# zju3dv/neuralbody

Hardware: NVIDIA H100
Metric: rays_per_s_512x512_64spp (higher is better)
Workload: dtype f16x2 (hi+lo fp16 pairs, fp32 accumulate)

## Files before the change

### neuralbody_b200/csrc/nb_render_tc_list.cu

```cuda
#include "nb_tc_common.cuh"
#include <type_traits>

namespace nb {
namespace tcl {

using tcr::Quad;

constexpr int TP = 128;
constexpr int NUM_SEGS = 6;
constexpr int MAXS = 1024;
constexpr uint32_t ID_MASK = 0x0FFFFFFFu;

__device__ __forceinline__ unsigned long long global_ns() {
    unsigned long long t;
    asm volatile("mov.u64 %0, %%globaltimer;" : "=l"(t));
    return t;
}

__device__ __forceinline__ void load_frame_xf(const RenderParams& P, FrameXf* xf, int i) {
    const int b = P.frame;
    if (i < 9) xf->R[i] = __ldg(P.R + b * 9 + i);
    if (i < 3) {
        xf->Th[i] = __ldg(P.Th + b * 3 + i);
        xf->min_dhw[i] = __ldg(P.bounds + b * 6 + (2 - i));
// ... 61 lines not shown
#pragma unroll
        for (int c = 0; c < 4; ++c) {
            const uint32_t bal = __ballot_sync(0xffffffffu, cls[k] == c);
            if (lane == 0) wcnt[c][slot] = __popc(bal);
        }
    }
    __syncthreads();
    if (tid < 4) {
        int total = 0;
        for (int w = 0; w < MAXS / 32; ++w) total += wcnt[tid][w];
        stotal[tid] = total;
        sbase[tid] = total ? atomicAdd(P.list_count + tid, (unsigned int)total) : 0u;
    }
    __syncthreads();
    const float4 empty = make_float4(0.f, 0.f, 0.f, fminf(sigma_empty, 0.f));
#pragma unroll
    for (int k = 0; k < CLS_PER_THREAD; ++k) {
        const int slot = k * (CLS_THREADS / 32) + warp;
        const int c = cls[k];
        const uint32_t same = __match_any_sync(0xffffffffu, c);
        if (c >= 0) {
            int local = __popc(same & ((1u << lane) - 1));
            for (int w = 0; w < slot; ++w) local += wcnt[c][w];
            float4* buf = c >= 2 ? P.list_a : P.list_b;
            const size_t at = (c & 1) ? (size_t)sbase[c] + local : P.list_cap - (size_t)sbase[c] - stotal[c] + local;
            buf[at] = gm[k];
        } else if (live[k]) {
            P.raw_ws[(__float_as_uint(gm[k].w) & ID_MASK) - id0] = empty;
        }
    }
}

constexpr int NT = 384;
constexpr int NROWT = 96;
constexpr int LAUNCH_REGS = (65536 / NT) / 8 * 8;
constexpr int PRODUCER_REGS = 56, CONSUMER_REGS = 224;
constexpr int CHUNK_STRIDE = TP * 16 + 16;
constexpr int ACT_CHUNKS = kHidden / 8;
constexpr int PLANE_BYTES = ACT_CHUNKS * CHUNK_STRIDE;
constexpr int SEG_BUFS = 4;
constexpr int SLOT_BYTES = 16384, NUM_SLOTS = 4;
constexpr int TILE256 = kHalfTile256 * 2;
constexpr int TILE3 = kHalfTile3 * 2;
constexpr int L3_PUSH = 4;
constexpr int L3_PUSHES = (kStepsL3 + L3_PUSH - 1) / L3_PUSH;
constexpr int HEAD_FLOATS = kHidden + 4 + 3 * kColor + 4 + 3 * kHidden;
constexpr int H_ALPHA = 0, H_RGBW = kHidden + 4, H_RGBB = H_RGBW + 3 * kColor, H_B0 = H_RGBB + 4;
constexpr int OFF_HI = 0, OFF_LO = PLANE_BYTES;
constexpr int OFF_RING = 2 * PLANE_BYTES;
constexpr int OFF_HEAD = OFF_RING + NUM_SLOTS * SLOT_BYTES;
constexpr int OFF_XF = OFF_HEAD + HEAD_FLOATS * 4;
constexpr int OFF_SCHED = OFF_XF + 128;
constexpr int OFF_ROWS = OFF_SCHED + 64;
constexpr int OFF_BAR = OFF_ROWS + 2 * TP * 16;
enum { B_FULL = 0, B_EMPTY = B_FULL + NUM_SLOTS, B_ROWSFULL = B_EMPTY + NUM_SLOTS, B_L2DONE, B_PEFULL, NUM_BARS };
constexpr int SMEM_BYTES = OFF_BAR + NUM_BARS * 8;
static_assert(SMEM_BYTES <= 232448, "shared memory budget");
static_assert(OFF_RING % 128 == 0 && OFF_HEAD % 16 == 0 && OFF_ROWS % 16 == 0 && OFF_BAR % 8 == 0, "alignment");
static_assert(128 * PRODUCER_REGS + 256 * CONSUMER_REGS <= NT * LAUNCH_REGS, "register pool of the CTA");

__host__ __device__ constexpr int pushes_per_tile(int l0_ksteps) { return l0_ksteps + 2 * kKsL12 + L3_PUSHES; }

__device__ __forceinline__ uint32_t act_off(int row, int k) {
    return (uint32_t)((k >> 3) * CHUNK_STRIDE + (row >> 3) * 128 + (row & 7) * 16 + (k & 7) * 2);
}

template <int NP, typename VT>
__global__ void __launch_bounds__(NT, 1) render_tc_list_kernel(const __grid_constant__ RenderParams P) {
    extern __shared__ __align__(1024) unsigned char smem[];
    uint64_t* bars = reinterpret_cast<uint64_t*>(smem + OFF_BAR);
    FrameXf* xf = reinterpret_cast<FrameXf*>(smem + OFF_XF);
    float* head = reinterpret_cast<float*>(smem + OFF_HEAD);
    float4* rows_buf = reinterpret_cast<float4*>(smem + OFF_ROWS);
    const int tid = threadIdx.x, lane = tid & 31;
    const int warp = __shfl_sync(0xffffffffu, tid >> 5, 0);
    const int wgid = warp >> 2;
    const int S = P.n_samples;
    const uint32_t s_hi0 = tc::smem_u32(smem + OFF_HI), s_lo0 = tc::smem_u32(smem + OFF_LO), s_ring = tc::smem_u32(smem + OFF_RING);

    if (tid == 0) {
        for (int i = 0; i < NUM_SLOTS; ++i) {
            tc::mbar_init(&bars[B_FULL + i], 1);
            tc::mbar_init(&bars[B_EMPTY + i], 8);
        }
        tc::mbar_init(&bars[B_ROWSFULL], NROWT);
        tc::mbar_init(&bars[B_L2DONE], 8);
        tc::mbar_init(&bars[B_PEFULL], NROWT);
        tc::fence_mbar_init();
    }
    load_frame_xf(P, xf, tid);
    for (int i = tid; i < HEAD_FLOATS; i += NT) {
        float v;
        if (i < H_RGBW) v = __ldg(P.wf32 + oAlphaW + i);
        else if (i < H_B0) v = __ldg(P.wf32 + oRgbW + (i - H_RGBW));
        else {
            const int j = i - H_B0, l = j / kHidden, n = j % kHidden;
            v = __ldg(P.wf32 + (l == 0 ? oB0 : l == 1 ? oB1 : oB2) + n);
        }
        head[i] = v;
    }
    struct Sched { unsigned int cnt[4]; int start[4]; int n_tiles; };
    Sched* sched = reinterpret_cast<Sched*>(smem + OFF_SCHED);
    if (tid == 0) {
        int acc = 0;
        for (int c = 0; c < 4; ++c) {
            const unsigned int n = P.list_count[c];
            sched->cnt[c] = n;
            sched->start[c] = acc;
            acc += (int)((n + TP - 1) / TP);
        }
        sched->n_tiles = acc;
        if (P.stats) atomicMax(P.frame_clock + 0, ~global_ns());
    }
    __syncthreads();
    const int n_tiles = sched->n_tiles;
    struct TileRef { int cls, nrows; const float4* ent; };
    auto tile_ref = [&](int tile) {
        TileRef r;
        r.cls = tile >= sched->start[3] ? 3 : tile >= sched->start[2] ? 2 : tile >= sched->start[1] ? 1 : 0;
        const int lt = tile - sched->start[r.cls];
        const unsigned int cnt = sched->cnt[r.cls];
        const long long rem = (long long)cnt - (long long)lt * TP;
        r.nrows = rem <= 0 ? 0 : rem < TP ? (int)rem : TP;
        const float4* buf = r.cls >= 2 ? P.list_a : P.list_b;
        r.ent = buf + ((r.cls & 1) ? (size_t)0 : P.list_cap - (size_t)cnt) + (size_t)lt * TP;
        return r;
    };

    if (wgid == 0) {
        tc::setmaxnreg_dec<PRODUCER_REGS>();
        const uint32_t s_hi = s_hi0, s_lo = s_lo0;
        if (warp == 0) {
            if (lane == 0) {
                tcr::Tracer tl;
                tl.init(P.trace, 3);
                const unsigned char* seq = reinterpret_cast<const unsigned char*>(P.wf16);
                unsigned long long real_tiles = 0, real_ksteps = 0;
                uint32_t g = 0;
                for (int tile = blockIdx.x; tile < n_tiles; tile += gridDim.x) {
                    const TileRef tref = tile_ref(tile);
                    const int l0_ksteps = class_ksteps(tref.cls);
                    real_tiles += tref.nrows > 0;
                    real_ksteps += tref.nrows > 0 ? l0_ksteps : 0;
                    for (int j = 0; j < pushes_per_tile(l0_ksteps); ++j, ++g) {
                        const uint32_t slot = g % NUM_SLOTS;
                        tc::mbar_wait(&bars[B_EMPTY + slot], ((g / NUM_SLOTS) & 1) ^ 1);
                        if (j == 0) tl.ev(1);
                        unsigned char* dst = smem + OFF_RING + slot * SLOT_BYTES;
                        uint64_t* bar = &bars[B_FULL + slot];
                        if (j < l0_ksteps + 2 * kKsL12) {
                            const int layer = j < l0_ksteps ? 0 : j < l0_ksteps + kKsL12 ? 1 : 2;
                            const int ks = layer == 0 ? j : layer == 1 ? j - l0_ksteps : j - l0_ksteps - kKsL12;
                            const int nks = layer == 0 ? kKsL0 : kKsL12;
                            const unsigned char* base = seq + 2 * (layer == 0 ? sL0 : layer == 1 ? sL1 : sL2);
                            tc::mbar_arrive_expect_tx(bar, (uint32_t)(2 * (NP == 3 ? 2 : 1) * TILE256));
#pragma unroll
                            for (int h = 0; h < 2; ++h)
#pragma unroll
                                for (int pl = 0; pl < (NP == 3 ? 2 : 1); ++pl)
                                    tc::bulk_g2s(dst + (2 * h + pl) * TILE256, base + 2 * pair_step_offset(ks, pl, h, nks), TILE256, bar);
                        } else {
                            const int g0 = (j - l0_ksteps - 2 * kKsL12) * L3_PUSH;
                            const int n = min(L3_PUSH, kStepsL3 - g0), common = min(n, kStepsL3 - 1 - g0);
                            const bool last = g0 + n == kStepsL3;
                            tc::mbar_arrive_expect_tx(bar, (uint32_t)(2 * n * TILE3));
#pragma unroll
                            for (int h = 0; h < 2; ++h) {
                                unsigned char* d = dst + h * (SLOT_BYTES / 2);
                                tc::bulk_g2s(d, seq + 2 * (sL3 + pair_l3_offset(g0, h)), common * TILE3, bar);
                                if (last)
                                    tc::bulk_g2s(d + common * TILE3, reinterpret_cast<const unsigned char*>(P.wframe) + ((size_t)P.frame * 2 + h) * TILE3,
                                                 TILE3, bar);
                            }
                        }
                    }
                    tl.ev(2);
                }
                if (P.stats) {
                    atomicAdd(P.stats + 0, real_tiles);
                    atomicAdd(P.stats + 4, real_ksteps);
                    if (blockIdx.x == 0) atomicAdd(P.stats + 1, (unsigned long long)sched->cnt[0] + sched->cnt[1] + sched->cnt[2] + sched->cnt[3]);
                }
            }
            __syncwarp();
        } else {
            const int pt = tid - 32;
            tcr::Tracer tr;
            tr.init(pt == 0 ? P.trace : nullptr, 0);
            auto pwait = [&](uint64_t* bar, uint32_t parity) { tc::mbar_wait_backoff(bar, parity, 64); };
            auto load_rows = [&](float4* dst, int tile) {
                if (tile < n_tiles) {
                    const TileRef r = tile_ref(tile);
                    for (int i = pt; i < TP; i += NROWT)
                        dst[i] = i < r.nrows ? __ldg(r.ent + i) : make_float4(0.f, 0.f, 0.f, __uint_as_float(0xFFFFFFFFu));
                }
                tcr::named_bar_sync(3, NROWT);
                tc::mbar_arrive(&bars[B_ROWSFULL]);
            };

            load_rows(rows_buf, blockIdx.x);
            int it = 0;
            for (int tile = blockIdx.x; tile < n_tiles; tile += gridDim.x, ++it) {
                const TileRef tref = tile_ref(tile);
                const int nrows = tref.nrows;
                const float4* rows = rows_buf + (it & 1) * TP;
                tr.ev(1);

                pwait(&bars[B_L2DONE], it & 1);
                tr.ev(31);
#pragma unroll 1
                for (int job = pt; job < 2 * TP; job += NROWT) {
                    const int prow = job % TP;
                    const float4 e = rows[prow];
                    auto put = [&](int k, float v) {
                        const __half hv = __float2half_rn(v);
                        asm volatile("st.shared.b16 [%0], %1;" ::"r"(s_lo + act_off(prow, k)), "h"(*reinterpret_cast<const unsigned short*>(&hv)) : "memory");
                    };
                    if (job < TP) {
                        positional_embed_anchored<10, 5>(e.x, e.y, e.z, [&](int j, float v) { put(j, v); });
                        put(63, 0.f);
                    } else {
                        const int smp = (int)(__float_as_uint(e.w) & ID_MASK);
                        const size_t ri = (size_t)P.frame * P.n_rays + (prow < nrows ? smp / S : 0);
                        const float dx = __ldg(P.ray_d + ri * 3), dy = __ldg(P.ray_d + ri * 3 + 1), dz = __ldg(P.ray_d + ri * 3 + 2);
                        const float nrm = sqrtf(__fadd_rn(__fadd_rn(__fmul_rn(dx, dx), __fmul_rn(dy, dy)), __fmul_rn(dz, dz)));
                        positional_embed_anchored<4, 4>(__fdiv_rn(dx, nrm), __fdiv_rn(dy, nrm), __fdiv_rn(dz, nrm), [&](int j, float v) { put(64 + j, v); });
                        put(91, 0.f); put(92, 1.f); put(93, 1.f); put(94, 0.f); put(95, 0.f);
                    }
                }
                tc::fence_proxy_async();
                tc::mbar_arrive(&bars[B_PEFULL]);
                tr.ev(32);
                load_rows(rows_buf + ((it + 1) & 1) * TP, tile + gridDim.x);
                tr.ev(30);
            }
        }
    } else {
        tc::setmaxnreg_inc<CONSUMER_REGS>();
        uint32_t s_hi, s_lo;
        const int cw = wgid - 1;
        const bool arr = lane == 0;
        tcr::Tracer tr;
        tr.init((tid & 127) == 0 ? P.trace : nullptr, 1 + cw);
        const int r0 = 64 * cw + 16 * (warp & 3) + (lane >> 2), cq = 2 * (lane & 3);
        float acc0[64], acc1[64];
        auto init_bias = [&](const float* b) {
#pragma unroll
            for (int c = 0; c < 16; ++c) {
                const float2 v0 = *reinterpret_cast<const float2*>(b + 8 * c + cq), v1 = *reinterpret_cast<const float2*>(b + 128 + 8 * c + cq);
                acc0[4 * c] = v0.x; acc0[4 * c + 1] = v0.y; acc0[4 * c + 2] = v0.x; acc0[4 * c + 3] = v0.y;
                acc1[4 * c] = v1.x; acc1[4 * c + 1] = v1.y; acc1[4 * c + 2] = v1.x; acc1[4 * c + 3] = v1.y;
            }
        };
        const uint32_t wg_rows = (uint32_t)(cw * 8 * 128);
        auto mma256 = [&](uint32_t slot, int ka) {
            const uint64_t a_hi = tc::make_smem_desc(s_hi + wg_rows + 2 * ka * CHUNK_STRIDE, CHUNK_STRIDE, 128);
            const uint64_t a_lo = tc::make_smem_desc(s_lo + wg_rows + 2 * ka * CHUNK_STRIDE, CHUNK_STRIDE, 128);
            const uint64_t b0h = tc::make_smem_desc(slot + 0 * TILE256, 128 * 16, 128);
            const uint64_t b0l = tc::make_smem_desc(slot + 1 * TILE256, 128 * 16, 128);
            const uint64_t b1h = tc::make_smem_desc(slot + 2 * TILE256, 128 * 16, 128);
            const uint64_t b1l = tc::make_smem_desc(slot + 3 * TILE256, 128 * 16, 128);
            tc::wgmma_m64n128k16_f16(acc0, a_hi, b0h, true);
            tc::wgmma_m64n128k16_f16(acc1, a_hi, b1h, true);
            if (NP == 3) {
                tc::wgmma_m64n128k16_f16(acc0, a_lo, b0h, true);
                tc::wgmma_m64n128k16_f16(acc1, a_lo, b1h, true);
                tc::wgmma_m64n128k16_f16(acc0, a_hi, b0l, true);
                tc::wgmma_m64n128k16_f16(acc1, a_hi, b1l, true);
            }
        };
        uint32_t g = 0;
        uint32_t w_stall = 0, r_stall = 0, pe_stall = 0, g_cycles = 0;
        auto take = [&](auto&& mma) {
            const uint32_t s = g % NUM_SLOTS;
            const uint32_t t0 = (uint32_t)clock();
            tc::mbar_wait(&bars[B_FULL + s], (g / NUM_SLOTS) & 1);
            w_stall += (uint32_t)clock() - t0;
            tc::wgmma_fence();
            mma(s_ring + s * SLOT_BYTES);
            tc::wgmma_commit();
            ++g;
        };
        auto release = [&](uint32_t gp, bool pred) { tc::mbar_arrive_if(&bars[B_EMPTY + gp % NUM_SLOTS], pred); };
        auto release_last = [&]() { release(g - 1, arr); };

        auto convert = [&](bool last) {
            float sig0 = 0.f, sig1 = 0.f;
            auto one = [&](const float (&a)[64], int nh) {
#pragma unroll
                for (int c = 0; c < 16; ++c) {
                    const int col = 128 * nh + 8 * c + cq;
#pragma unroll
                    for (int hr = 0; hr < 2; ++hr) {
                        const float x0 = a[4 * c + 2 * hr], x1 = a[4 * c + 2 * hr + 1];
                        const uint32_t off = act_off(r0 + 8 * hr, col);
                        uint32_t hv;
                        if (last) {
                            const float2 aw = *reinterpret_cast<const float2*>(head + H_ALPHA + col);
                            float& sg = hr ? sig1 : sig0;
                            sg = fmaf(fmaxf(x0, 0.f), aw.x, sg);
                            sg = fmaf(fmaxf(x1, 0.f), aw.y, sg);
                            hv = tc::cvt_relu_f16x2(x0, x1);
                        } else if (NP == 3) {
                            hv = tc::cvt_rz_relu_f16x2(x0, x1);
                            float q0, q1;
                            tc::trunc_residual2(x0, x1, q0, q1);
                            const uint32_t lv = tc::cvt_relu_f16x2(q0, q1);
                            asm volatile("st.shared.b32 [%0], %1;" ::"r"(s_lo + off), "r"(lv) : "memory");
                        } else {
                            hv = tc::cvt_relu_f16x2(x0, x1);
                        }
                        asm volatile("st.shared.b32 [%0], %1;" ::"r"(s_hi + off), "r"(hv) : "memory");
                    }
                }
            };
            one(acc0, 0);
            one(acc1, 1);
            return make_float2(sig0, sig1);
        };
        auto publish = [&]() {
            tc::fence_proxy_async();
            tcr::named_bar_sync(1 + cw, 128);
        };

        int it = 0;
        for (int tile = blockIdx.x; tile < n_tiles; tile += gridDim.x, ++it) {
            const TileRef tref = tile_ref(tile);
            const int nrows = tref.nrows, nseg = class_segments(tref.cls);
            const float4* rows = rows_buf + (it & 1) * TP;
            asm volatile("mov.u32 %0, %1;" : "=r"(s_hi) : "r"(s_hi0));
            asm volatile("mov.u32 %0, %1;" : "=r"(s_lo) : "r"(s_lo0));
            tr.ev(1);
            auto gather = [&](int seg) {
                const unsigned char* volbase = reinterpret_cast<const unsigned char*>(P.volume);
                const int grp = (tid & 127) >> 3, t = tid & 7;
                const int lvl = seg < 2 ? 3 : seg < 4 ? 2 : seg < 5 ? 1 : 0;
                const int cbase0 = seg < 2 ? seg * 64 : seg < 4 ? (seg - 2) * 64 : 0;
                const int nunits = seg == NUM_SEGS - 1 ? 1 : 2;
                const int C = P.lvl_C[lvl], D = P.lvl_D[lvl], H = P.lvl_H[lvl], W = P.lvl_W[lvl];
                const unsigned char* lvl_ptr = volbase + P.lvl_off[lvl] + ((size_t)P.frame * P.lvl_bstride[lvl] + 4 * t) * sizeof(VT);
                const uint32_t dX = (uint32_t)(C * sizeof(VT)), dY = dX * W, dZ = dY * H;
                const int kb = 64 * (seg % SEG_BUFS);
                for (int row = 64 * cw + grp; row < 64 * cw + 64; row += 16) {
                    const float4 e = rows[row];
                    const bool occ = row < nrows && ((__float_as_uint(e.w) >> (28 + lvl)) & 1u);
                    float acc[2][4] = {{0.f, 0.f, 0.f, 0.f}, {0.f, 0.f, 0.f, 0.f}};
                    if (occ) {
                        float gx, gy, gz;
                        world_to_grid(*xf, e.x, e.y, e.z, gx, gy, gz);
                        Corners cn;
                        corner_setup(unnormalize(gx, W), unnormalize(gy, H), unnormalize(gz, D), W, H, D, cn);
                        auto axis = [](int i0, int size, float (&w)[2]) {
                            if (i0 < 0) { w[0] = w[1]; w[1] = 0.f; return 0; }
                            if (i0 >= size) { w[0] = w[1] = 0.f; return size - 2; }
                            if (i0 == size - 1) { w[1] = w[0]; w[0] = 0.f; return size - 2; }
                            return i0;
                        };
                        const int xc = axis(cn.x0, W, cn.wx), yc = axis(cn.y0, H, cn.wy), zc = axis(cn.z0, D, cn.wz);
                        const uint32_t cb = (uint32_t)((zc * H + yc) * W + xc) * dX;
                        float cw[8];
#pragma unroll
                        for (int c = 0; c < 8; ++c) cw[c] = __fmul_rn(__fmul_rn(cn.wx[c & 1], cn.wy[(c >> 1) & 1]), cn.wz[c >> 2]);
#pragma unroll
                        for (int uu = 0; uu < 2; ++uu) {
                            if (uu >= nunits) continue;
                            const unsigned char* ub = lvl_ptr + (size_t)(cbase0 + 32 * uu) * sizeof(VT);
                            typename Quad<VT>::raw v[8];
#pragma unroll
                            for (int c = 0; c < 8; ++c)
                                v[c] = Quad<VT>::load_bytes(ub + cb + ((c & 1) ? dX : 0u) + ((c & 2) ? dY : 0u) + ((c & 4) ? dZ : 0u));
#pragma unroll
                            for (int c = 0; c < 8; ++c)
                                if (cw[c] != 0.f) Quad<VT>::fma(acc[uu], v[c], cw[c]);
                        }
                    }
#pragma unroll
                    for (int uu = 0; uu < 2; ++uu) {
                        if (uu >= nunits) continue;
                        const float (&a)[4] = acc[uu];
                        const uint32_t off = act_off(row, kb + 32 * uu + 4 * t);
                        uint2 hw, lw;
                        if (NP == 3) {
                            hw.x = tc::cvt_rz_f16x2(a[0], a[1]); hw.y = tc::cvt_rz_f16x2(a[2], a[3]);
                            float q0, q1, q2, q3;
                            tc::trunc_residual2(a[0], a[1], q0, q1);
                            tc::trunc_residual2(a[2], a[3], q2, q3);
                            lw.x = tc::cvt_f16x2(q0, q1); lw.y = tc::cvt_f16x2(q2, q3);
                            tcr::sts_v2(s_lo + off, lw);
                        } else {
                            hw.x = tc::cvt_f16x2(a[0], a[1]); hw.y = tc::cvt_f16x2(a[2], a[3]);
                        }
                        tcr::sts_v2(s_hi + off, hw);
                    }
                }
            };

            {
                const uint32_t t0 = (uint32_t)clock();
                tc::mbar_wait(&bars[B_ROWSFULL], it & 1);
                r_stall += (uint32_t)clock() - t0;
            }
            init_bias(head + H_B0);
            for (int seg = 0; seg < nseg; ++seg) {
                const uint32_t t0 = (uint32_t)clock();
                gather(seg);
                publish();
                g_cycles += (uint32_t)clock() - t0;
                const int nks = seg == NUM_SEGS - 1 ? 2 : 4, ka = 4 * (seg % SEG_BUFS);
                for (int q = 0; q < nks; ++q) {
                    take([&](uint32_t slot) { mma256(slot, ka + q); });
                    tc::wgmma_wait<1>();
                    tc::acc_fence(acc0); tc::acc_fence(acc1);
                    release(g - 2, arr && q > 0);
                }
                tc::wgmma_wait<0>();
                tc::acc_fence(acc0); tc::acc_fence(acc1);
                release_last();
            }
            tr.ev(20);
            convert(false);
            init_bias(head + H_B0 + kHidden);
            publish();
            float2 sig = make_float2(0.f, 0.f);
            for (int layer = 1; layer <= 2; ++layer) {
                for (int q = 0; q < kKsL12; ++q) {
                    take([&](uint32_t slot) { mma256(slot, q); });
                    tc::wgmma_wait<1>();
                    tc::acc_fence(acc0); tc::acc_fence(acc1);
                    release(g - 2, arr && q > 0);
                }
                tc::wgmma_wait<0>();
                tc::acc_fence(acc0); tc::acc_fence(acc1);
                release_last();
                tr.ev(20 + layer);
                if (layer == 1) {
                    convert(false);
                    init_bias(head + H_B0 + 2 * kHidden);
                } else {
                    tc::mbar_arrive_if(&bars[B_L2DONE], arr);
                    sig = convert(true);
                }
                publish();
            }
            float c3a[32], c3b[32];
#pragma unroll
            for (int i = 0; i < 32; ++i) { c3a[i] = 0.f; c3b[i] = 0.f; }
#pragma unroll
            for (int p = 0; p < L3_PUSHES; ++p) {
                if (p * L3_PUSH == 16) {
                    const uint32_t t0 = (uint32_t)clock();
                    tc::mbar_wait(&bars[B_PEFULL], it & 1);
                    pe_stall += (uint32_t)clock() - t0;
                }
                take([&](uint32_t slot) {
#pragma unroll
                    for (int k = 0; k < L3_PUSH; ++k) {
                        const int ks = p * L3_PUSH + k;
                        if (ks >= kStepsL3) break;
                        const uint32_t a = ks < 16 ? s_hi + 2 * ks * CHUNK_STRIDE : s_lo + 2 * (ks - 16) * CHUNK_STRIDE;
                        const uint64_t ad = tc::make_smem_desc(a + wg_rows, CHUNK_STRIDE, 128);
                        tc::wgmma_m64n64k16_f16(c3a, ad, tc::make_smem_desc(slot + k * TILE3, 64 * 16, 128), true);
                        tc::wgmma_m64n64k16_f16(c3b, ad, tc::make_smem_desc(slot + SLOT_BYTES / 2 + k * TILE3, 64 * 16, 128), true);
                    }
                });
                tc::wgmma_wait<1>();
                tc::acc_fence(c3a); tc::acc_fence(c3b);
                release(g - 2, arr && p > 0);
            }
            tc::wgmma_wait<0>();
            tc::acc_fence(c3a); tc::acc_fence(c3b);
            release_last();
            tr.ev(23);
            float cr[2] = {0.f, 0.f}, cg[2] = {0.f, 0.f}, cbl[2] = {0.f, 0.f};
            auto color = [&](const float (&a)[32], int nh) {
#pragma unroll
                for (int c = 0; c < 8; ++c) {
                    const int col = 64 * nh + 8 * c + cq;
                    const float2 w0 = *reinterpret_cast<const float2*>(head + H_RGBW + col);
                    const float2 w1 = *reinterpret_cast<const float2*>(head + H_RGBW + kColor + col);
                    const float2 w2 = *reinterpret_cast<const float2*>(head + H_RGBW + 2 * kColor + col);
#pragma unroll
                    for (int hr = 0; hr < 2; ++hr) {
                        const float x0 = fmaxf(a[4 * c + 2 * hr], 0.f), x1 = fmaxf(a[4 * c + 2 * hr + 1], 0.f);
                        cr[hr] = fmaf(x1, w0.y, fmaf(x0, w0.x, cr[hr]));
                        cg[hr] = fmaf(x1, w1.y, fmaf(x0, w1.x, cg[hr]));
                        cbl[hr] = fmaf(x1, w2.y, fmaf(x0, w2.x, cbl[hr]));
                    }
                }
            };
            color(c3a, 0);
            color(c3b, 1);
            float sg[2] = {sig.x, sig.y};
#pragma unroll
            for (int hr = 0; hr < 2; ++hr) {
#pragma unroll
                for (int o = 1; o <= 2; o <<= 1) {
                    cr[hr] += __shfl_xor_sync(0xffffffffu, cr[hr], o);
                    cg[hr] += __shfl_xor_sync(0xffffffffu, cg[hr], o);
                    cbl[hr] += __shfl_xor_sync(0xffffffffu, cbl[hr], o);
                    sg[hr] += __shfl_xor_sync(0xffffffffu, sg[hr], o);
                }
                const int row = r0 + 8 * hr;
                if ((lane & 3) == 0 && row < nrows) {
                    const int smp = (int)(__float_as_uint(rows[row].w) & ID_MASK);
                    P.raw_ws[smp] = make_float4(cr[hr] + head[H_RGBB], cg[hr] + head[H_RGBB + 1], cbl[hr] + head[H_RGBB + 2],
                                                sg[hr] + head[H_ALPHA + kHidden]);
                }
            }
            tr.ev(24);
            tr.val(50, w_stall);
            tr.val(51, r_stall);
            tr.val(52, pe_stall);
            tr.val(53, g_cycles);
            w_stall = r_stall = pe_stall = g_cycles = 0;
        }
    }
    __syncthreads();
    if (tid == 0 && P.stats) atomicMax(P.frame_clock + 1, global_ns());
}

constexpr int COMP_WARPS = 8;
__global__ void __launch_bounds__(COMP_WARPS * 32) composite_kernel(const __grid_constant__ RenderParams P) {
    __shared__ float zs[COMP_WARPS][MAXS];
    const int warp = threadIdx.x >> 5, lane = threadIdx.x & 31;
    const int ray = blockIdx.x * COMP_WARPS + warp;
    if (blockIdx.x == 0 && threadIdx.x == 0 && P.stats) {
        const unsigned long long t0 = ~P.frame_clock[0], t1 = P.frame_clock[1];
        atomicAdd(P.stats + 2, t1 > t0 ? t1 - t0 : 0ull);
        atomicAdd(P.stats + 3, 1ull);
    }
    if (ray >= P.n_rays) return;
    const int S = P.n_samples;
    const size_t rg = (size_t)P.frame * P.n_rays + ray;
    const float near = __ldg(P.near + rg), far = __ldg(P.far + rg);
    for (int s = lane; s < S; s += 32) zs[warp][s] = z_sample(near, far, P.t_vals, s, S, P.t_rand ? P.t_rand + rg * S : nullptr, P.z_user ? P.z_user + rg * S : nullptr);
    __syncwarp();
    const float dx = __ldg(P.ray_d + rg * 3), dy = __ldg(P.ray_d + rg * 3 + 1), dz = __ldg(P.ray_d + rg * 3 + 2);
    const float nrm = sqrtf(__fadd_rn(__fadd_rn(__fmul_rn(dx, dx), __fmul_rn(dy, dy)), __fmul_rn(dz, dz)));
    float* wout = P.weights ? P.weights + rg * S : nullptr;
    RayOut o = composite_ray(P.raw_ws + (size_t)ray * S, zs[warp], S, nrm, wout, lane);
    if (lane == 0) {
        const float add = P.white_bkgd ? __fsub_rn(1.f, o.acc) : 0.f;
        P.rgb_map[rg * P.rgb_stride + 0] = o.r + add;
        P.rgb_map[rg * P.rgb_stride + 1] = o.g + add;
        P.rgb_map[rg * P.rgb_stride + 2] = o.b + add;
        P.depth_map[rg * P.map_stride] = o.depth;
        P.acc_map[rg * P.map_stride] = o.acc;
        P.disp_map[rg * P.map_stride] = disparity(o.depth, o.acc);
    }
}

template <int NP, typename VT>
static cudaError_t launch_list(const RenderParams& p, int grid, cudaStream_t stream) {
    cudaError_t e = cudaFuncSetAttribute(render_tc_list_kernel<NP, VT>, cudaFuncAttributeMaxDynamicSharedMemorySize, SMEM_BYTES);
    if (e != cudaSuccess) return e;
    render_tc_list_kernel<NP, VT><<<grid, NT, SMEM_BYTES, stream>>>(p);
    return cudaGetLastError();
}

static size_t align256(size_t v) { return (v + 255) & ~(size_t)255; }
constexpr size_t CTL_BYTES = 32;

}

bool tc_available() { return true; }

size_t render_tc_list_workspace_bytes(int batch, int n_rays, int n_samples) {
    const size_t per_frame = (size_t)n_rays * n_samples * sizeof(float4);
    return tcl::align256((size_t)batch * tcl::CTL_BYTES) + 3 * tcl::align256(per_frame);
}

// ... 70 lines not shown
```

### neuralbody_b200/csrc/nb_tc_common.cuh

```cuda
#pragma once
#include "nb_device.cuh"
#include "nb_tc_ptx.cuh"

namespace nb {
namespace tcr {

__device__ __forceinline__ void named_bar_sync(int id, int nthreads) {
    asm volatile("bar.sync %0, %1;" ::"r"(id), "r"(nthreads) : "memory");
}
__device__ __forceinline__ uint4 ldg_nc_v4(const void* p) {
    uint4 r;
    asm volatile("ld.global.nc.v4.u32 {%0,%1,%2,%3}, [%4];" : "=r"(r.x), "=r"(r.y), "=r"(r.z), "=r"(r.w) : "l"(p));
    return r;
}
__device__ __forceinline__ void sts_v2(uint32_t addr, uint2 v) {
    asm volatile("st.shared.v2.b32 [%0], {%1, %2};" ::"r"(addr), "r"(v.x), "r"(v.y) : "memory");
}
__device__ __forceinline__ float f16lo_of(float x, uint32_t hi_pair, int which) {
    const __half2 h = *reinterpret_cast<const __half2*>(&hi_pair);
    return x - (which ? __high2float(h) : __low2float(h));
}

struct Tracer {
    unsigned long long* buf;
    int n;
    __device__ __forceinline__ void init(unsigned long long* base, int role) {
        buf = (base && blockIdx.x == 0) ? base + role * 4096 : nullptr;
        n = 0;
    }
    __device__ __forceinline__ void ev(int code) { val(code, (unsigned long long)clock64()); }
    __device__ __forceinline__ void val(int code, unsigned long long v) {
        if (buf && n < 4096) buf[n++] = ((unsigned long long)code << 48) | (v & 0xFFFFFFFFFFFFull);
    }
};

template <typename VT> struct Quad;
template <> struct Quad<float> {
    using raw = uint4;
    static __device__ __forceinline__ raw zero() { return make_uint4(0u, 0u, 0u, 0u); }
    static __device__ __forceinline__ raw load(const float* p) { return ldg_nc_v4(p); }
    static __device__ __forceinline__ raw load_bytes(const unsigned char* p) { return ldg_nc_v4(p); }
    static __device__ __forceinline__ void fma(float (&a)[4], const raw& v, float w) {
        a[0] = fmaf(__uint_as_float(v.x), w, a[0]); a[1] = fmaf(__uint_as_float(v.y), w, a[1]);
        a[2] = fmaf(__uint_as_float(v.z), w, a[2]); a[3] = fmaf(__uint_as_float(v.w), w, a[3]);
    }
};
template <> struct Quad<__half> {
    using raw = uint2;
    static __device__ __forceinline__ raw zero() { return make_uint2(0u, 0u); }
    static __device__ __forceinline__ raw load(const __half* p) {
        uint2 r;
        asm volatile("ld.global.nc.v2.u32 {%0,%1}, [%2];" : "=r"(r.x), "=r"(r.y) : "l"(p));
        return r;
    }
    static __device__ __forceinline__ raw load_bytes(const unsigned char* p) { return load(reinterpret_cast<const __half*>(p)); }
    static __device__ __forceinline__ void fma(float (&a)[4], const raw& v, float w) {
        const float2 f0 = __half22float2(*reinterpret_cast<const __half2*>(&v.x));
        const float2 f1 = __half22float2(*reinterpret_cast<const __half2*>(&v.y));
        a[0] = fmaf(f0.x, w, a[0]); a[1] = fmaf(f0.y, w, a[1]);
        a[2] = fmaf(f1.x, w, a[2]); a[3] = fmaf(f1.y, w, a[3]);
    }
};

}
}
```

### neuralbody_b200/csrc/nb_tc_ptx.cuh

```cuda
#pragma once
#include <cuda_fp16.h>
#include <stdint.h>

namespace nb {
namespace tc {

__device__ __forceinline__ uint32_t smem_u32(const void* p) { return (uint32_t)__cvta_generic_to_shared(p); }

__device__ __forceinline__ void mbar_init(uint64_t* bar, uint32_t count) {
    asm volatile("mbarrier.init.shared::cta.b64 [%0], %1;" ::"r"(smem_u32(bar)), "r"(count));
}
__device__ __forceinline__ void fence_mbar_init() { asm volatile("fence.mbarrier_init.release.cluster;" ::: "memory"); }
__device__ __forceinline__ void mbar_arrive(uint64_t* bar) {
    asm volatile("{\n\t.reg .b64 st;\n\tmbarrier.arrive.shared::cta.b64 st, [%0];\n\t}" ::"r"(smem_u32(bar)) : "memory");
}
__device__ __forceinline__ void mbar_arrive_if(uint64_t* bar, bool pred) {
    asm volatile("{\n\t.reg .pred p;\n\t.reg .b64 st;\n\tsetp.ne.b32 p, %1, 0;\n\t@p mbarrier.arrive.shared::cta.b64 st, [%0];\n\t}" ::"r"(
                     smem_u32(bar)),
                 "r"((uint32_t)pred)
                 : "memory");
}
template <int N>
__device__ __forceinline__ void setmaxnreg_dec() { asm volatile("setmaxnreg.dec.sync.aligned.u32 %0;" ::"n"(N)); }
template <int N>
// ... 6 lines not shown
__device__ __forceinline__ bool mbar_try_wait(uint64_t* bar, uint32_t parity) {
    uint32_t ok;
    asm volatile(
        "{\n\t.reg .pred p;\n\t"
#ifdef NB_NO_WAIT_HINT
        "mbarrier.try_wait.parity.shared::cta.b64 p, [%1], %2;\n\t"
#else
        "mbarrier.try_wait.parity.shared::cta.b64 p, [%1], %2, 1000000;\n\t"
#endif
        "selp.u32 %0, 1, 0, p;\n\t}"
        : "=r"(ok)
        : "r"(smem_u32(bar)), "r"(parity)
        : "memory");
    return ok != 0;
}
#ifndef NB_WATCHDOG_PROBES
#define NB_WATCHDOG_PROBES 20000u
#endif
__device__ __forceinline__ void mbar_wait(uint64_t* bar, uint32_t parity) {
    uint32_t probes = 0;
    while (!mbar_try_wait(bar, parity)) {
        if (++probes > NB_WATCHDOG_PROBES) __trap();
    }
}

__device__ __forceinline__ bool mbar_test(uint64_t* bar, uint32_t parity) {
    uint32_t ok;
    asm volatile(
        "{\n\t.reg .pred p;\n\t"
        "mbarrier.test_wait.parity.shared::cta.b64 p, [%1], %2;\n\t"
        "selp.u32 %0, 1, 0, p;\n\t}"
        : "=r"(ok)
        : "r"(smem_u32(bar)), "r"(parity)
        : "memory");
    return ok != 0;
}

__device__ __forceinline__ void mbar_wait_backoff(uint64_t* bar, uint32_t parity, unsigned ns) {
    uint32_t probes = 0;
    while (!mbar_try_wait(bar, parity)) {
        __nanosleep(ns);
        if (++probes > NB_WATCHDOG_PROBES * 64u) __trap();
    }
}

__device__ __forceinline__ void fence_proxy_async() { asm volatile("fence.proxy.async.shared::cta;" ::: "memory"); }

__device__ __forceinline__ void bulk_g2s(void* smem_dst, const void* gmem_src, uint32_t bytes, uint64_t* bar) {
    asm volatile("cp.async.bulk.shared::cluster.global.mbarrier::complete_tx::bytes [%0], [%1], %2, [%3];" ::"r"(
                     smem_u32(smem_dst)),
                 "l"(gmem_src), "r"(bytes), "r"(smem_u32(bar))
                 : "memory");
}

__device__ __forceinline__ uint64_t make_smem_desc(uint32_t smem_addr, uint32_t lbo_bytes, uint32_t sbo_bytes) {
    uint64_t d = 0;
    d |= (uint64_t)((smem_addr & 0x3FFFFu) >> 4);
    d |= (uint64_t)((lbo_bytes >> 4) & 0x3FFFu) << 16;
    d |= (uint64_t)((sbo_bytes >> 4) & 0x3FFFu) << 32;
    return d;
}
__device__ __forceinline__ uint64_t desc_add(uint64_t d, uint32_t bytes) { return d + (uint64_t)(bytes >> 4); }

__device__ __forceinline__ void wgmma_fence() { asm volatile("wgmma.fence.sync.aligned;" ::: "memory"); }
__device__ __forceinline__ void wgmma_commit() { asm volatile("wgmma.commit_group.sync.aligned;" ::: "memory"); }
template <int N>
__device__ __forceinline__ void wgmma_wait() { asm volatile("wgmma.wait_group.sync.aligned %0;" ::"n"(N) : "memory"); }

__device__ __forceinline__ void wgmma_m64n128k16_f16(float (&d)[64], uint64_t a_desc, uint64_t b_desc, bool accumulate) {
    asm volatile(
        "{\n\t.reg .pred p;\n\tsetp.ne.b32 p, %66, 0;\n\t"
        "wgmma.mma_async.sync.aligned.m64n128k16.f32.f16.f16 "
        "{"
        "%0,%1,%2,%3,%4,%5,%6,%7,%8,%9,%10,%11,%12,%13,%14,%15,%16,%17,%18,%19,%20,%21,%22,%23,%24,%25,%26,%2"
        "7,%28,%29,%30,%31,%32,%33,%34,%35,%36,%37,%38,%39,%40,%41,%42,%43,%44,%45,%46,%47,%48,%49,%50,%51,%5"
        "2,%53,%54,%55,%56,%57,%58,%59,%60,%61,%62,%63"
        "}, %64, %65, p, 1, 1, 0, 0;\n\t}"
        : "+f"(d[0]), "+f"(d[1]), "+f"(d[2]), "+f"(d[3]), "+f"(d[4]), "+f"(d[5]), "+f"(d[6]), "+f"(d[7]), "+f"(d[8]), "+f"(d[9]), "+f"(d[10]), "+f"(d[11]), "+f"(d[12]), "+f"(d[13]), "+f"(d[14]), "+f"(d[15]), "+f"(d[16]), "+f"(d[17]), "+f"(d[18]), "+f"(d[19]), "+f"(d[20]), "+f"(d[21]), "+f"(d[22]), "+f"(d[23]), "+f"(d[24]), "+f"(d[25]), "+f"(d[26]), "+f"(d[27]), "+f"(d[28]), "+f"(d[29]), "+f"(d[30]), "+f"(d[31]), "+f"(d[32]), "+f"(d[33]), "+f"(d[34]), "+f"(d[35]), "+f"(d[36]), "+f"(d[37]), "+f"(d[38]), "+f"(d[39]), "+f"(d[40]), "+f"(d[41]), "+f"(d[42]), "+f"(d[43]), "+f"(d[44]), "+f"(d[45]), "+f"(d[46]), "+f"(d[47]), "+f"(d[48]), "+f"(d[49]), "+f"(d[50]), "+f"(d[51]), "+f"(d[52]), "+f"(d[53]), "+f"(d[54]), "+f"(d[55]), "+f"(d[56]), "+f"(d[57]), "+f"(d[58]), "+f"(d[59]), "+f"(d[60]), "+f"(d[61]), "+f"(d[62]), "+f"(d[63])
        : "l"(a_desc), "l"(b_desc), "r"((uint32_t)accumulate)
        : "memory");
}

__device__ __forceinline__ void wgmma_m64n64k16_f16(float (&d)[32], uint64_t a_desc, uint64_t b_desc, bool accumulate) {
    asm volatile(
        "{\n\t.reg .pred p;\n\tsetp.ne.b32 p, %34, 0;\n\t"
        "wgmma.mma_async.sync.aligned.m64n64k16.f32.f16.f16 "
        "{"
        "%0,%1,%2,%3,%4,%5,%6,%7,%8,%9,%10,%11,%12,%13,%14,%15,%16,%17,%18,%19,%20,%21,%22,%23,%24,%25,%26,%2"
        "7,%28,%29,%30,%31"
        "}, %32, %33, p, 1, 1, 0, 0;\n\t}"
        : "+f"(d[0]), "+f"(d[1]), "+f"(d[2]), "+f"(d[3]), "+f"(d[4]), "+f"(d[5]), "+f"(d[6]), "+f"(d[7]), "+f"(d[8]), "+f"(d[9]), "+f"(d[10]), "+f"(d[11]), "+f"(d[12]), "+f"(d[13]), "+f"(d[14]), "+f"(d[15]), "+f"(d[16]), "+f"(d[17]), "+f"(d[18]), "+f"(d[19]), "+f"(d[20]), "+f"(d[21]), "+f"(d[22]), "+f"(d[23]), "+f"(d[24]), "+f"(d[25]), "+f"(d[26]), "+f"(d[27]), "+f"(d[28]), "+f"(d[29]), "+f"(d[30]), "+f"(d[31])
        : "l"(a_desc), "l"(b_desc), "r"((uint32_t)accumulate)
        : "memory");
}

__device__ __forceinline__ void wgmma_m64n256k8_tf32(float (&d)[128], uint64_t a_desc, uint64_t b_desc, bool accumulate) {
    asm volatile(
        "{\n\t.reg .pred p;\n\tsetp.ne.b32 p, %130, 0;\n\t"
        "wgmma.mma_async.sync.aligned.m64n256k8.f32.tf32.tf32 "
        "{"
        "%0,%1,%2,%3,%4,%5,%6,%7,%8,%9,%10,%11,%12,%13,%14,%15,%16,%17,%18,%19,%20,%21,%22,%23,%24,%25,%26,%2"
        "7,%28,%29,%30,%31,%32,%33,%34,%35,%36,%37,%38,%39,%40,%41,%42,%43,%44,%45,%46,%47,%48,%49,%50,%51,%5"
        "2,%53,%54,%55,%56,%57,%58,%59,%60,%61,%62,%63,%64,%65,%66,%67,%68,%69,%70,%71,%72,%73,%74,%75,%76,%7"
        "7,%78,%79,%80,%81,%82,%83,%84,%85,%86,%87,%88,%89,%90,%91,%92,%93,%94,%95,%96,%97,%98,%99,%100,%101,"
        "%102,%103,%104,%105,%106,%107,%108,%109,%110,%111,%112,%113,%114,%115,%116,%117,%118,%119,%120,%121,"
        "%122,%123,%124,%125,%126,%127"
// ... 47 lines not shown
```

Baseline: 13.44 million.

## Stage deduplicated coarse-level voxels in shared memory for trilinear gather

Producer warps now build a per-tile hash table of the unique voxel corners touched by each 64-row half for the coarse levels, and remap per-row corner slots to compact indices. Consumers cp.async those unique voxel feature vectors into spare activation-plane space and perform the trilinear blend from shared memory instead of issuing 8 scattered global loads per row; they fall back to the global path when a tile touches more than the capacity. Row loading and table building are moved ahead, gated by a new rows-free barrier, so they overlap the previous tile. This adds hashing atomics, extra shared memory and synchronization, and aims to cut redundant global gather traffic.

```diff
diff --git a/neuralbody_b200/csrc/nb_render_tc_list.cu b/neuralbody_b200/csrc/nb_render_tc_list.cu
--- a/neuralbody_b200/csrc/nb_render_tc_list.cu
+++ b/neuralbody_b200/csrc/nb_render_tc_list.cu
@@ -137,17 +137,45 @@
 constexpr int OFF_XF = OFF_HEAD + HEAD_FLOATS * 4;
 constexpr int OFF_SCHED = OFF_XF + 128;
 constexpr int OFF_ROWS = OFF_SCHED + 64;
-constexpr int OFF_BAR = OFF_ROWS + 2 * TP * 16;
-enum { B_FULL = 0, B_EMPTY = B_FULL + NUM_SLOTS, B_ROWSFULL = B_EMPTY + NUM_SLOTS, B_L2DONE, B_PEFULL, NUM_BARS };
+constexpr int NV = 64;
+constexpr int NTAB = 4;
+constexpr int HBITS = 7, HSIZE = 1 << HBITS;
+constexpr uint32_t HEMPTY = 0xFFFFFFFFu;
+constexpr int kCoarseC = 128;
+struct VoxTable {
+    unsigned char slot[TP][2][8];
+    uint32_t ids[NTAB][NV];
+    uint32_t n[NTAB];
+};
+constexpr int OFF_VTAB = OFF_ROWS + 2 * TP * 16;
+constexpr int OFF_HKEY = OFF_VTAB + 2 * (int)sizeof(VoxTable);
+constexpr int OFF_HVAL = OFF_HKEY + NTAB * HSIZE * 4;
+constexpr int OFF_HCNT = OFF_HVAL + NTAB * HSIZE;
+constexpr int OFF_BAR = OFF_HCNT + (NTAB + 2) * 4;
+enum { B_FULL = 0, B_EMPTY = B_FULL + NUM_SLOTS, B_ROWSFULL = B_EMPTY + NUM_SLOTS, B_L2DONE, B_PEFULL, B_ROWSFREE, NUM_BARS };
 constexpr int SMEM_BYTES = OFF_BAR + NUM_BARS * 8;
 static_assert(SMEM_BYTES <= 232448, "shared memory budget");
-static_assert(OFF_RING % 128 == 0 && OFF_HEAD % 16 == 0 && OFF_ROWS % 16 == 0 && OFF_BAR % 8 == 0, "alignment");
+static_assert(OFF_RING % 128 == 0 && OFF_HEAD % 16 == 0 && OFF_ROWS % 16 == 0 && OFF_VTAB % 16 == 0 && OFF_HKEY % 16 == 0 &&
+              OFF_BAR % 8 == 0, "alignment");
+static_assert(NV * kCoarseC * 4 <= 2 * 2 * 8 * 1024 && NV <= 255 && HSIZE > NV, "voxel staging");
 static_assert(128 * PRODUCER_REGS + 256 * CONSUMER_REGS <= NT * LAUNCH_REGS, "register pool of the CTA");
 
 __host__ __device__ constexpr int pushes_per_tile(int l0_ksteps) { return l0_ksteps + 2 * kKsL12 + L3_PUSHES; }
 
 __device__ __forceinline__ uint32_t act_off(int row, int k) {
     return (uint32_t)((k >> 3) * CHUNK_STRIDE + (row >> 3) * 128 + (row & 7) * 16 + (k & 7) * 2);
+}
+
+__device__ __forceinline__ uint32_t clamped_cell(float gx, float gy, float gz, int W, int H, int D, Corners& cn) {
+    corner_setup(unnormalize(gx, W), unnormalize(gy, H), unnormalize(gz, D), W, H, D, cn);
+    auto axis = [](int i0, int size, float (&w)[2]) {
+        if (i0 < 0) { w[0] = w[1]; w[1] = 0.f; return 0; }
+        if (i0 >= size) { w[0] = w[1] = 0.f; return size - 2; }
+        if (i0 == size - 1) { w[1] = w[0]; w[0] = 0.f; return size - 2; }
+        return i0;
+    };
+    const int xc = axis(cn.x0, W, cn.wx), yc = axis(cn.y0, H, cn.wy), zc = axis(cn.z0, D, cn.wz);
+    return (uint32_t)((zc * H + yc) * W + xc);
 }
 
 template <int NP, typename VT>
@@ -171,6 +199,7 @@
         tc::mbar_init(&bars[B_ROWSFULL], NROWT);
         tc::mbar_init(&bars[B_L2DONE], 8);
         tc::mbar_init(&bars[B_PEFULL], NROWT);
+        tc::mbar_init(&bars[B_ROWSFREE], 8);
         tc::fence_mbar_init();
     }
     load_frame_xf(P, xf, tid);
@@ -184,6 +213,8 @@
         }
         head[i] = v;
     }
+    for (int i = tid; i < NTAB * HSIZE; i += NT) reinterpret_cast<uint32_t*>(smem + OFF_HKEY)[i] = HEMPTY;
+    if (tid < NTAB + 2) reinterpret_cast<uint32_t*>(smem + OFF_HCNT)[tid] = 0u;
     struct Sched { unsigned int cnt[4]; int start[4]; int n_tiles; };
     Sched* sched = reinterpret_cast<Sched*>(smem + OFF_SCHED);
     if (tid == 0) {
@@ -270,27 +301,103 @@
             __syncwarp();
         } else {
             const int pt = tid - 32;
+            VoxTable* vtabs = reinterpret_cast<VoxTable*>(smem + OFF_VTAB);
+            uint32_t* hkey = reinterpret_cast<uint32_t*>(smem + OFF_HKEY);
+            unsigned char* hval = smem + OFF_HVAL;
+            uint32_t* hcnt = reinterpret_cast<uint32_t*>(smem + OFF_HCNT);
             tcr::Tracer tr;
             tr.init(pt == 0 ? P.trace : nullptr, 0);
             auto pwait = [&](uint64_t* bar, uint32_t parity) { tc::mbar_wait_backoff(bar, parity, 64); };
-            auto load_rows = [&](float4* dst, int tile) {
+            auto insert = [&](int tab, uint32_t id, VoxTable* vt) -> uint32_t {
+                if (*reinterpret_cast<volatile uint32_t*>(hcnt + tab) > (uint32_t)NV) return 0xFFu;
+                uint32_t* keys = hkey + tab * HSIZE;
+                uint32_t h = (id * 2654435761u) >> (32 - HBITS);
+#pragma unroll 1
+                for (int p = 0; p < HSIZE; ++p, h = (h + 1) & (HSIZE - 1)) {
+                    uint32_t k = *reinterpret_cast<volatile uint32_t*>(keys + h);
+                    if (k == HEMPTY) k = atomicCAS(keys + h, HEMPTY, id);
+                    if (k == HEMPTY) {
+                        const uint32_t s = atomicAdd(hcnt + tab, 1u);
+                        if (s < (uint32_t)NV) vt->ids[tab][s] = id;
+                        hval[tab * HSIZE + h] = (unsigned char)min(s, 255u);
+                        return h;
+                    }
+                    if (k == id) return h;
+                }
+                return 0xFFu;
+            };
+            auto build_table = [&](VoxTable* vt, const float4* rows, int nrows, int nlev) {
+#pragma unroll 1
+                for (int row = pt; row < TP; row += NROWT) {
+                    const float4 e = rows[row];
+                    float gx, gy, gz;
+                    world_to_grid(*xf, e.x, e.y, e.z, gx, gy, gz);
+#pragma unroll 1
+                    for (int li = 0; li < nlev; ++li) {
+                        const int lvl = 3 - li, tab = 2 * (row >> 6) + li;
+                        uint32_t w[2] = {0xFFFFFFFFu, 0xFFFFFFFFu};
+                        if (row < nrows && ((__float_as_uint(e.w) >> (28 + lvl)) & 1u)) {
+                            const int D = P.lvl_D[lvl], H = P.lvl_H[lvl], W = P.lvl_W[lvl];
+                            Corners cn;
+                            const uint32_t base = clamped_cell(gx, gy, gz, W, H, D, cn);
+#pragma unroll
+                            for (int c = 0; c < 8; ++c) {
+                                const uint32_t id = base + ((c & 1) ? 1u : 0u) + ((c & 2) ? (uint32_t)W : 0u) + ((c & 4) ? (uint32_t)(W * H) : 0u);
+                                const uint32_t h = insert(tab, id, vt);
+                                w[c >> 2] = (w[c >> 2] & ~(0xFFu << (8 * (c & 3)))) | (h << (8 * (c & 3)));
+                            }
+                        }
+                        *reinterpret_cast<uint2*>(&vt->slot[row][li][0]) = make_uint2(w[0], w[1]);
+                    }
+                }
+                tcr::named_bar_sync(3, NROWT);
+                uint32_t* words = reinterpret_cast<uint32_t*>(&vt->slot[0][0][0]);
+#pragma unroll 1
+                for (int i = pt; i < TP * 2 * 2; i += NROWT) {
+                    const int li = (i >> 1) & 1;
+                    if (li >= nlev) continue;
+                    const unsigned char* hv = hval + (2 * ((i >> 2) >> 6) + li) * HSIZE;
+                    uint32_t wd = words[i], out = 0u;
+#pragma unroll
+                    for (int b = 0; b < 4; ++b) {
+                        const uint32_t h = (wd >> (8 * b)) & 0xFFu;
+                        out |= (h == 0xFFu ? 0xFFu : (uint32_t)hv[h]) << (8 * b);
+                    }
+                    words[i] = out;
+                }
+                for (int i = pt; i < NTAB * HSIZE; i += NROWT) hkey[i] = HEMPTY;
+                if (pt < NTAB) {
+                    const uint32_t n = hcnt[pt];
+                    vt->n[pt] = n;
+                    hcnt[pt] = 0u;
+                    if ((pt & 1) < nlev && nrows > 64 * (pt >> 1)) atomicAdd(hcnt + NTAB + (n <= (uint32_t)NV ? 0 : 1), 1u);
+                }
+            };
+            auto load_rows = [&](int buf, int tile) {
                 if (tile < n_tiles) {
                     const TileRef r = tile_ref(tile);
+                    float4* dst = rows_buf + buf * TP;
                     for (int i = pt; i < TP; i += NROWT)
                         dst[i] = i < r.nrows ? __ldg(r.ent + i) : make_float4(0.f, 0.f, 0.f, __uint_as_float(0xFFFFFFFFu));
+                    tcr::named_bar_sync(3, NROWT);
+                    build_table(vtabs + buf, dst, r.nrows, class_segments(r.cls) >= 4 ? 2 : 1);
                 }
                 tcr::named_bar_sync(3, NROWT);
                 tc::mbar_arrive(&bars[B_ROWSFULL]);
             };
 
-            load_rows(rows_buf, blockIdx.x);
-            int it = 0;
-            for (int tile = blockIdx.x; tile < n_tiles; tile += gridDim.x, ++it) {
+            int it = -1;
+            for (int tile = (int)blockIdx.x - (int)gridDim.x; tile < n_tiles; tile += gridDim.x, ++it) {
+                if (it >= 0) {
+                    pwait(&bars[B_ROWSFREE], it & 1);
+                    tr.ev(1);
+                }
+                load_rows((it + 1) & 1, tile + gridDim.x);
+                if (it < 0) continue;
+                tr.ev(30);
                 const TileRef tref = tile_ref(tile);
                 const int nrows = tref.nrows;
                 const float4* rows = rows_buf + (it & 1) * TP;
-                tr.ev(1);
-
                 pwait(&bars[B_L2DONE], it & 1);
                 tr.ev(31);
 #pragma unroll 1
@@ -316,8 +423,6 @@
                 tc::fence_proxy_async();
                 tc::mbar_arrive(&bars[B_PEFULL]);
                 tr.ev(32);
-                load_rows(rows_buf + ((it + 1) & 1) * TP, tile + gridDim.x);
-                tr.ev(30);
             }
         }
     } else {
@@ -325,8 +430,11 @@
         uint32_t s_hi, s_lo;
         const int cw = wgid - 1;
         const bool arr = lane == 0;
-        tcr::Tracer tr;
-        tr.init((tid & 127) == 0 ? P.trace : nullptr, 1 + cw);
+        int tn = ((tid & 127) == 0 && blockIdx.x == 0 && P.trace) ? (1 + cw) * 4096 : -1;
+        auto tval = [&](int code, unsigned long long v) {
+            if (tn >= 0 && tn < (2 + cw) * 4096) P.trace[tn++] = ((unsigned long long)code << 48) | (v & 0xFFFFFFFFFFFFull);
+        };
+        auto tev = [&](int code) { tval(code, (unsigned long long)clock64()); };
         const int r0 = 64 * cw + 16 * (warp & 3) + (lane >> 2), cq = 2 * (lane & 3);
         float acc0[64], acc1[64];
         auto init_bias = [&](const float* b) {
@@ -415,37 +523,90 @@
             const float4* rows = rows_buf + (it & 1) * TP;
             asm volatile("mov.u32 %0, %1;" : "=r"(s_hi) : "r"(s_hi0));
             asm volatile("mov.u32 %0, %1;" : "=r"(s_lo) : "r"(s_lo0));
-            tr.ev(1);
+            tev(1);
             auto gather = [&](int seg) {
                 const unsigned char* volbase = reinterpret_cast<const unsigned char*>(P.volume);
+                const VoxTable* vt = reinterpret_cast<const VoxTable*>(smem + OFF_VTAB) + (it & 1);
                 const int grp = (tid & 127) >> 3, t = tid & 7;
                 const int lvl = seg < 2 ? 3 : seg < 4 ? 2 : seg < 5 ? 1 : 0;
                 const int cbase0 = seg < 2 ? seg * 64 : seg < 4 ? (seg - 2) * 64 : 0;
                 const int nunits = seg == NUM_SEGS - 1 ? 1 : 2;
                 const int C = P.lvl_C[lvl], D = P.lvl_D[lvl], H = P.lvl_H[lvl], W = P.lvl_W[lvl];
-                const unsigned char* lvl_ptr = volbase + P.lvl_off[lvl] + ((size_t)P.frame * P.lvl_bstride[lvl] + 4 * t) * sizeof(VT);
-                const uint32_t dX = (uint32_t)(C * sizeof(VT)), dY = dX * W, dZ = dY * H;
                 const int kb = 64 * (seg % SEG_BUFS);
-                for (int row = 64 * cw + grp; row < 64 * cw + 64; row += 16) {
-                    const float4 e = rows[row];
-                    const bool occ = row < nrows && ((__float_as_uint(e.w) >> (28 + lvl)) & 1u);
-                    float acc[2][4] = {{0.f, 0.f, 0.f, 0.f}, {0.f, 0.f, 0.f, 0.f}};
-                    if (occ) {
-                        float gx, gy, gz;
-                        world_to_grid(*xf, e.x, e.y, e.z, gx, gy, gz);
-                        Corners cn;
-                        corner_setup(unnormalize(gx, W), unnormalize(gy, H), unnormalize(gz, D), W, H, D, cn);
-                        auto axis = [](int i0, int size, float (&w)[2]) {
-                            if (i0 < 0) { w[0] = w[1]; w[1] = 0.f; return 0; }
-                            if (i0 >= size) { w[0] = w[1] = 0.f; return size - 2; }
-                            if (i0 == size - 1) { w[1] = w[0]; w[0] = 0.f; return size - 2; }
-                            return i0;
-                        };
-                        const int xc = axis(cn.x0, W, cn.wx), yc = axis(cn.y0, H, cn.wy), zc = axis(cn.z0, D, cn.wz);
-                        const uint32_t cb = (uint32_t)((zc * H + yc) * W + xc) * dX;
-                        float cw[8];
-#pragma unroll
-                        for (int c = 0; c < 8; ++c) cw[c] = __fmul_rn(__fmul_rn(cn.wx[c & 1], cn.wy[(c >> 1) & 1]), cn.wz[c >> 2]);
+                constexpr uint32_t VB = kCoarseC * sizeof(VT), VPP = 1024 / VB, PPV = VB / 16;
+                const int tab = 2 * cw + (seg >> 1);
+                const bool staged = seg < 4 && C == kCoarseC && vt->n[tab] <= (uint32_t)NV;
+                const uint32_t st_base = s_hi + (seg < 2 ? 16 : 0) * CHUNK_STRIDE + cw * 1024;
+                auto stage_addr = [&](uint32_t v) {
+                    const uint32_t p = v / VPP;
+                    return st_base + (p >> 4) * PLANE_BYTES + (p & 15) * CHUNK_STRIDE + (v % VPP) * VB;
+                };
+                if (staged && (seg & 1) == 0) {
+                    const unsigned char* src = volbase + P.lvl_off[lvl] + (size_t)P.frame * P.lvl_bstride[lvl] * sizeof(VT);
+                    const uint32_t nq = vt->n[tab] * PPV;
+#pragma unroll 4
+                    for (uint32_t i = tid & 127; i < nq; i += 128) {
+                        const uint32_t v = i / PPV, q = i % PPV;
+                        tc::cp_async_16(stage_addr(v) + 16 * q, src + (size_t)vt->ids[tab][v] * VB + 16 * q);
+                    }
+                    tc::cp_async_wait_all();
+                    tcr::named_bar_sync(1 + cw, 128);
+                }
+                auto rows_loop = [&](auto&& blend) {
+                    for (int row = 64 * cw + grp; row < 64 * cw + 64; row += 16) {
+                        const float4 e = rows[row];
+                        const bool occ = row < nrows && ((__float_as_uint(e.w) >> (28 + lvl)) & 1u);
+                        float acc[2][4] = {{0.f, 0.f, 0.f, 0.f}, {0.f, 0.f, 0.f, 0.f}};
+                        if (occ) {
+                            float gx, gy, gz;
+                            world_to_grid(*xf, e.x, e.y, e.z, gx, gy, gz);
+                            Corners cn;
+                            const uint32_t cb = clamped_cell(gx, gy, gz, W, H, D, cn);
+                            float cw[8];
+#pragma unroll
+                            for (int c = 0; c < 8; ++c) cw[c] = __fmul_rn(__fmul_rn(cn.wx[c & 1], cn.wy[(c >> 1) & 1]), cn.wz[c >> 2]);
+                            blend(row, cb, cw, acc);
+                        }
+#pragma unroll
+                        for (int uu = 0; uu < 2; ++uu) {
+                            if (uu >= nunits) continue;
+                            const float (&a)[4] = acc[uu];
+                            const uint32_t off = act_off(row, kb + 32 * uu + 4 * t);
+                            uint2 hw, lw;
+                            if (NP == 3) {
+                                hw.x = tc::cvt_rz_f16x2(a[0], a[1]); hw.y = tc::cvt_rz_f16x2(a[2], a[3]);
+                                float q0, q1, q2, q3;
+                                tc::trunc_residual2(a[0], a[1], q0, q1);
+                                tc::trunc_residual2(a[2], a[3], q2, q3);
+                                lw.x = tc::cvt_f16x2(q0, q1); lw.y = tc::cvt_f16x2(q2, q3);
+                                tcr::sts_v2(s_lo + off, lw);
+                            } else {
+                                hw.x = tc::cvt_f16x2(a[0], a[1]); hw.y = tc::cvt_f16x2(a[2], a[3]);
+                            }
+                            tcr::sts_v2(s_hi + off, hw);
+                        }
+                    }
+                };
+                if (staged) {
+                    const uint32_t st_off = ((seg & 1) * 64 + 4 * t) * sizeof(VT);
+                    const int li = seg >> 1;
+                    rows_loop([&](int row, uint32_t, const float (&cw)[8], float (&acc)[2][4]) {
+                        const uint2 sl = *reinterpret_cast<const uint2*>(&vt->slot[row][li][0]);
+#pragma unroll
+                        for (int c = 0; c < 8; ++c) {
+                            const uint32_t a = stage_addr((((c < 4) ? sl.x : sl.y) >> (8 * (c & 3))) & 0xFFu) + st_off;
+                            const typename Quad<VT>::raw v0 = Quad<VT>::load_shared(a), v1 = Quad<VT>::load_shared(a + 32 * sizeof(VT));
+                            if (cw[c] != 0.f) {
+                                Quad<VT>::fma(acc[0], v0, cw[c]);
+                                Quad<VT>::fma(acc[1], v1, cw[c]);
+                            }
+                        }
+                    });
+                } else {
+                    const unsigned char* lvl_ptr = volbase + P.lvl_off[lvl] + ((size_t)P.frame * P.lvl_bstride[lvl] + 4 * t) * sizeof(VT);
+                    const uint32_t dX = (uint32_t)(C * sizeof(VT)), dY = dX * W, dZ = dY * H;
+                    rows_loop([&](int, uint32_t cell, const float (&cw)[8], float (&acc)[2][4]) {
+                        const uint32_t cb = cell * dX;
 #pragma unroll
                         for (int uu = 0; uu < 2; ++uu) {
                             if (uu >= nunits) continue;
@@ -458,25 +619,7 @@
                             for (int c = 0; c < 8; ++c)
                                 if (cw[c] != 0.f) Quad<VT>::fma(acc[uu], v[c], cw[c]);
                         }
-                    }
-#pragma unroll
-                    for (int uu = 0; uu < 2; ++uu) {
-                        if (uu >= nunits) continue;
-                        const float (&a)[4] = acc[uu];
-                        const uint32_t off = act_off(row, kb + 32 * uu + 4 * t);
-                        uint2 hw, lw;
-                        if (NP == 3) {
-                            hw.x = tc::cvt_rz_f16x2(a[0], a[1]); hw.y = tc::cvt_rz_f16x2(a[2], a[3]);
-                            float q0, q1, q2, q3;
-                            tc::trunc_residual2(a[0], a[1], q0, q1);
-                            tc::trunc_residual2(a[2], a[3], q2, q3);
-                            lw.x = tc::cvt_f16x2(q0, q1); lw.y = tc::cvt_f16x2(q2, q3);
-                            tcr::sts_v2(s_lo + off, lw);
-                        } else {
-                            hw.x = tc::cvt_f16x2(a[0], a[1]); hw.y = tc::cvt_f16x2(a[2], a[3]);
-                        }
-                        tcr::sts_v2(s_hi + off, hw);
-                    }
+                    });
                 }
             };
 
@@ -485,6 +628,8 @@
                 tc::mbar_wait(&bars[B_ROWSFULL], it & 1);
                 r_stall += (uint32_t)clock() - t0;
             }
+            __syncwarp();
+            tc::mbar_arrive_if(&bars[B_ROWSFREE], arr);
             init_bias(head + H_B0);
             for (int seg = 0; seg < nseg; ++seg) {
                 const uint32_t t0 = (uint32_t)clock();
@@ -502,7 +647,7 @@
                 tc::acc_fence(acc0); tc::acc_fence(acc1);
                 release_last();
             }
-            tr.ev(20);
+            tev(20);
             convert(false);
             init_bias(head + H_B0 + kHidden);
             publish();
@@ -517,7 +662,7 @@
                 tc::wgmma_wait<0>();
                 tc::acc_fence(acc0); tc::acc_fence(acc1);
                 release_last();
-                tr.ev(20 + layer);
+                tev(20 + layer);
                 if (layer == 1) {
                     convert(false);
                     init_bias(head + H_B0 + 2 * kHidden);
@@ -555,7 +700,7 @@
             tc::wgmma_wait<0>();
             tc::acc_fence(c3a); tc::acc_fence(c3b);
             release_last();
-            tr.ev(23);
+            tev(23);
             float cr[2] = {0.f, 0.f}, cg[2] = {0.f, 0.f}, cbl[2] = {0.f, 0.f};
             auto color = [&](const float (&a)[32], int nh) {
 #pragma unroll
@@ -592,16 +737,21 @@
                                                 sg[hr] + head[H_ALPHA + kHidden]);
                 }
             }
-            tr.ev(24);
-            tr.val(50, w_stall);
-            tr.val(51, r_stall);
-            tr.val(52, pe_stall);
-            tr.val(53, g_cycles);
+            tev(24);
+            tval(50, w_stall);
+            tval(51, r_stall);
+            tval(52, pe_stall);
+            tval(53, g_cycles);
             w_stall = r_stall = pe_stall = g_cycles = 0;
         }
     }
     __syncthreads();
-    if (tid == 0 && P.stats) atomicMax(P.frame_clock + 1, global_ns());
+    if (tid == 0 && P.stats) {
+        atomicMax(P.frame_clock + 1, global_ns());
+        const uint32_t* paths = reinterpret_cast<const uint32_t*>(smem + OFF_HCNT) + NTAB;
+        atomicAdd(P.stats + 5, (unsigned long long)paths[0]);
+        atomicAdd(P.stats + 6, (unsigned long long)paths[1]);
+    }
 }
 
 constexpr int COMP_WARPS = 8;
diff --git a/neuralbody_b200/csrc/nb_tc_common.cuh b/neuralbody_b200/csrc/nb_tc_common.cuh
--- a/neuralbody_b200/csrc/nb_tc_common.cuh
+++ b/neuralbody_b200/csrc/nb_tc_common.cuh
@@ -40,6 +40,11 @@
     static __device__ __forceinline__ raw zero() { return make_uint4(0u, 0u, 0u, 0u); }
     static __device__ __forceinline__ raw load(const float* p) { return ldg_nc_v4(p); }
     static __device__ __forceinline__ raw load_bytes(const unsigned char* p) { return ldg_nc_v4(p); }
+    static __device__ __forceinline__ raw load_shared(uint32_t addr) {
+        uint4 r;
+        asm volatile("ld.shared.v4.u32 {%0,%1,%2,%3}, [%4];" : "=r"(r.x), "=r"(r.y), "=r"(r.z), "=r"(r.w) : "r"(addr) : "memory");
+        return r;
+    }
     static __device__ __forceinline__ void fma(float (&a)[4], const raw& v, float w) {
         a[0] = fmaf(__uint_as_float(v.x), w, a[0]); a[1] = fmaf(__uint_as_float(v.y), w, a[1]);
         a[2] = fmaf(__uint_as_float(v.z), w, a[2]); a[3] = fmaf(__uint_as_float(v.w), w, a[3]);
@@ -54,6 +59,11 @@
         return r;
     }
     static __device__ __forceinline__ raw load_bytes(const unsigned char* p) { return load(reinterpret_cast<const __half*>(p)); }
+    static __device__ __forceinline__ raw load_shared(uint32_t addr) {
+        uint2 r;
+        asm volatile("ld.shared.v2.u32 {%0,%1}, [%2];" : "=r"(r.x), "=r"(r.y) : "r"(addr) : "memory");
+        return r;
+    }
     static __device__ __forceinline__ void fma(float (&a)[4], const raw& v, float w) {
         const float2 f0 = __half22float2(*reinterpret_cast<const __half2*>(&v.x));
         const float2 f1 = __half22float2(*reinterpret_cast<const __half2*>(&v.y));
diff --git a/neuralbody_b200/csrc/nb_tc_ptx.cuh b/neuralbody_b200/csrc/nb_tc_ptx.cuh
--- a/neuralbody_b200/csrc/nb_tc_ptx.cuh
+++ b/neuralbody_b200/csrc/nb_tc_ptx.cuh
@@ -82,6 +82,11 @@
                  "l"(gmem_src), "r"(bytes), "r"(smem_u32(bar))
                  : "memory");
 }
+
+__device__ __forceinline__ void cp_async_16(uint32_t smem_dst, const void* gmem_src) {
+    asm volatile("cp.async.cg.shared.global [%0], [%1], 16;" ::"r"(smem_dst), "l"(gmem_src) : "memory");
+}
+__device__ __forceinline__ void cp_async_wait_all() { asm volatile("cp.async.wait_all;" ::: "memory"); }
 
 __device__ __forceinline__ uint64_t make_smem_desc(uint32_t smem_addr, uint32_t lbo_bytes, uint32_t sbo_bytes) {
     uint64_t d = 0;
```

Result: faster. 14.28 million (median of 6 runs) (+6.3%).
